# Xiaoming-Zhao/PointNav-VO

Measured on AMD Instinct MI355X. Metric: RGB-D frame-pair VO inferences/s @341x192, higher is better.
Workload: dtype f32

## Files before the change

pointnav-vo_amd/csrc/pnvo_api.hip:

```cpp
#include <hip/hip_runtime.h>

#include <cmath>
#include <cstdio>
#include <cstdlib>
#include <cstring>
#include <functional>
#include <atomic>
#include <condition_variable>
#include <map>
#include <mutex>
#include <string>
#include <thread>
#include <vector>

#include "pnvo_model.h"

using namespace pnvo;

thread_local std::string g_err;

int pnvo_fail(pnvo_handle h, int code, const std::string &msg) {
  if (h) h->err = msg;
  g_err = msg;
  return code;
// ... 432 lines not shown
void pnvo_drop_graphs(pnvo_handle m) {
  for (auto &g : m->graphs) {
    (void)hipGraphExecDestroy(g.exec);
    (void)hipGraphDestroy(g.graph);
  }
  m->graphs.clear();
  m->seen.clear();
}

void pnvo_chain_in_bounds(pnvo_handle h, const std::function<float(const Layer &)> &gn_bound) {
  if (h->bottleneck || h->convs.empty()) return;
  float bin = gn_bound(h->convs[0]);
  size_t li = 1;
  for (int stage = 1; stage <= 4; ++stage)
    for (int bi = 0; bi < h->nblocks[stage - 1]; ++bi) {
      if (li + 1 >= h->convs.size()) return;
      Layer &c1 = h->convs[li++];
      Layer &c2 = h->convs[li++];
      const bool ds = li < h->convs.size() && h->convs[li].name.find("downsample") != std::string::npos;
      c1.in_bound = bin;
      c2.in_bound = gn_bound(c1);
      float skip = bin;
      if (ds) {
        Layer &cd = h->convs[li++];
        cd.in_bound = bin;
        skip = gn_bound(cd);
      }
      bin = gn_bound(c2) + skip;
    }
  if (li < h->convs.size()) h->convs[li].in_bound = bin;
}

bool pnvo_conv_on_x3(pnvo_handle m, const Layer &l, int B) {
  if (!x3_layer(m, l) || l.groups <= 0) return false;
  ConvX3Args xa;
  int mw, nw;
  size_t ldsb;
  return x3_args(m, l, B, xa, &mw, &nw, &ldsb);
}

bool pnvo_conv_takes_ds(pnvo_handle m, const Layer &c1, const Layer &cd, int B) {
  if (!m->opt.ds_fuse || m->tap_dst != nullptr || m->bottleneck) return false;
  if (c1.k != 3 || c1.kw != 3 || c1.stride != 2 || c1.pad != 1 || cd.k != 1 || cd.kw != 1 || cd.stride != 2 || cd.pad != 0) return false;
  if (c1.cinp != cd.cinp || c1.coutp != cd.coutp || c1.cout != cd.cout || c1.hout != cd.hout || c1.wout != cd.wout || c1.hin != cd.hin ||
      c1.win != cd.win || c1.cout != c1.coutp || c1.groups != cd.groups || c1.groups <= 0 || cd.host_w.empty())
    return false;
  if (!x3_layer(m, c1) || !x3_layer(m, cd) || !x3_two_pieces(m, c1) || !x3_two_pieces(m, cd)) return false;
  return pnvo_conv_on_x3(m, c1, B);
}

bool pnvo_conv_takes_tail(pnvo_handle m, const Layer &l, int B) {
  if (m->tap_dst != nullptr || !m->opt.tail) return false;
  return pnvo_conv_on_x3(m, l, B);
}

namespace {
double conv_flops(const Layer &l, int B) { return 2.0 * ((double)((long)B * l.hout * l.wout) * l.cout * l.cin * l.k * l.kw); }
double conv_bytes(const Layer &l, int B) {
  return 4.0 * ((double)B * l.hin * l.win * l.cin + (double)((long)B * l.hout * l.wout) * l.cout + (double)l.cout * l.cin * l.k * l.kw);
}

int x3_operand(pnvo_handle h, Layer &q, int pieces, hipStream_t s) {
  unsigned short *&wpk = pieces == 2 ? q.wpk_x2 : q.wpk_x3;
  unsigned long long &gen = pieces == 2 ? q.x2_gen : q.x3_gen;
  if (wpk && gen == h->weights_gen) return PNVO_OK;
  const size_t nel = (size_t)q.k * q.kw * q.cinp * q.coutp * pieces;
  if (!wpk) HIPCHK(h, hipMalloc((void **)&wpk, nel * 2));
  const float *dev_w = h->train ? pnvo_train_weight_ptr(h, q.name + ".weight") : nullptr;
  if (dev_w != nullptr && pieces == 2) {
    HIPCHK(h, launch_conv_x2_repack(dev_w, q.cout, q.cin, q.cinp, q.coutp, q.k, q.kw, pnvo_train_x2_scale(h, q.name + ".weight"), wpk, s));
  } else if (dev_w != nullptr) {
    HIPCHK(h, launch_conv_x3_repack(dev_w, q.cout, q.cin, q.cinp, q.coutp, q.k, q.kw, 0, wpk, s));
  } else {
    std::vector<unsigned short> pk(nel);
    if (pieces == 2)
      q.x2_oscale = pack_conv_x2_weight(q.host_w.data(), q.cout, q.cin, q.cinp, q.coutp, q.k, q.kw, pk.data());
    else
      pack_conv_x3_weight(q.host_w.data(), q.cout, q.cin, q.cinp, q.coutp, q.k, q.kw, pk.data());
    HIPCHK(h, hipMemcpyAsync(wpk, pk.data(), nel * 2, hipMemcpyHostToDevice, s));
    HIPCHK(h, hipStreamSynchronize(s));
  }
  gen = h->weights_gen;
  return PNVO_OK;
}

int run_conv_x3(pnvo_handle m, const Layer &l, int B, const ConvRequest &r, ConvX3Args &xa, bool rows, int x3_mode, int mw, int nw,
                size_t ldsb) {
  hipStream_t s = r.s;
  const DsRide *ride = r.ride;
  const bool two = xa.np == 2;
  Layer &lm = const_cast<Layer &>(l);
  if (int rc = x3_operand(m, lm, xa.np, s)) return rc;
  if (ride != nullptr) {
    if (rows || !two || l.stride != 2 || l.k != 3) return fail(m, PNVO_ERR_STATE, "downsample ride on a conv that cannot carry it (" + l.name + ")");
    Layer &dm = const_cast<Layer &>(*ride->cd);
    if (int rc = x3_operand(m, dm, 2, s)) return rc;
    xa.ds_wpk = dm.wpk_x2;
    xa.ds_oscale = dm.x2_oscale;
    if (m->train != nullptr) {
      const float *sp = pnvo_train_x2_scale(m, dm.name + ".weight");
      xa.ds_oscale_ptr = sp ? sp + 1 : nullptr;
    }
    xa.ds_y = ride->y;
    xa.ds_stats = m->stats_ds;
  }
  GnGroup gg{0x7fffffff, 0x7fffffff, {nullptr, nullptr}, {nullptr, nullptr}}, ggd = gg;
// ... 448 lines not shown
    a.CPL = m->CPL;
    a.slots = stem_tiles_x(m->Ws) * stem_tiles_y(m->Hs);
    a.dbg = m->opt.stem_dbg;
    a.lds_pad = m->opt.stem_dbg_pad;
    const double M = (double)B * m->Hs * m->Ws;
    {
      Timed t(m, s, "conv:" + stem.name, 2.0 * M * stem.cout * stem.cin * 49,
              4.0 * ((double)B * c.height * c.width * stem.cin + M * stem.cout + (double)stem.cout * stem.cin * 49));
      HIPCHK(m, launch_stem_lds(a, stem.coutp, s));
    }
    m->stem_slots_out = a.slots;
    if (!skip_finalize) {
      Timed t(m, s, "gn_finalize", 0.0, 0.0);
      HIPCHK(m, launch_gn_finalize(m->stats, B, a.slots, stem.coutp, stem.cout, stem.groups, (long)m->Hs * m->Ws, 1,
                                   stem.gamma, stem.beta, 1e-5f, ss[0], ss[1], s, a.slots, mu_out, rstd_out));
    }
  } else {
    if ((rc = pnvo_run_conv(m, stem, B, {.in_scale = m->stem_sc, .in_shift = m->stem_sh, .y = y, .y_cstride = stem.coutp, .ss = ss,
                                         .mu = mu_out, .rstd = rstd_out, .src = src, .grp = grp, .s = s})) != PNVO_OK)
      return rc;
  }
  return rc;
}

int pnvo_ensure_workspace(pnvo_handle m, int B) { return ensure_workspace(m, B); }

namespace {
struct OptChoice {
  const char *word;
  int value;
};
struct OptDef {
  const char *key, *env;
  int PnvoOptions::*field;
  bool numeric;
  OptChoice choices[7];
};
const OptDef kOptions[] = {
    {"stem", "PNVO_STEM", &PnvoOptions::stem, false, {{"auto", 0}, {"mx", 1}, {"dd", 2}, {"dense", 3}, {nullptr, 0}}},
    {"conv", "PNVO_CONV", &PnvoOptions::conv, false, {{"auto", 0}, {"x3", 1}, {"fp32", 2}, {"generic", 3}, {nullptr, 0}}},
    {"pieces", "PNVO_PIECES", &PnvoOptions::pieces, false, {{"2", 2}, {"3", 3}, {nullptr, 0}}},
    {"stem_form", "PNVO_STEM_FORM", &PnvoOptions::stem_form, false, {{"auto", 0}, {"tiles", 2}, {"resident", 3}, {"fast", 4}, {nullptr, 0}}},
    {"train_pieces", "PNVO_TRAIN_PIECES", &PnvoOptions::train_pieces, false, {{"2", 2}, {"3", 3}, {nullptr, 0}}},
    {"x3_persist", "PNVO_X3_PERSIST", &PnvoOptions::x3_persist, false, {{"on", 1}, {"off", 0}, {nullptr, 0}}},
    {"x3_rows", "PNVO_X3_ROWS", &PnvoOptions::x3_rows, false, {{"on", 1}, {"off", 0}, {nullptr, 0}}},
    {"x3_strip", "PNVO_X3_STRIP", &PnvoOptions::x3_strip, false, {{"on", 1}, {"off", 0}, {nullptr, 0}}},
    {"x3_fine", "PNVO_X3_FINE", &PnvoOptions::x3_fine, false, {{"on", 1}, {"off", 0}, {nullptr, 0}}},
    {"x3_w8", "PNVO_X3_W8", &PnvoOptions::x3_w8, false, {{"on", 1}, {"off", 0}, {nullptr, 0}}},
    {"x3_ksplit", "PNVO_X3_KSPLIT", &PnvoOptions::x3_ksplit, false, {{"on", 1}, {"off", 0}, {nullptr, 0}}},
    {"fc_rows", "PNVO_FC_ROWS", &PnvoOptions::fc_rows, true, {{nullptr, 0}}},
    {"head_fuse", "PNVO_HEAD_FUSE", &PnvoOptions::head_fuse, false, {{"on", 1}, {"off", 0}, {nullptr, 0}}},
    {"ds_fuse", "PNVO_DS_FUSE", &PnvoOptions::ds_fuse, false, {{"on", 1}, {"off", 0}, {nullptr, 0}}},
    {"gn_fuse", "PNVO_GN_FUSE", &PnvoOptions::gn_fuse, false, {{"on", 1}, {"off", 0}, {nullptr, 0}}},
    {"x3_s2", nullptr, &PnvoOptions::x3_s2, false, {{"on", 1}, {"off", 0}, {nullptr, 0}}},
    {"tail", "PNVO_TAIL", &PnvoOptions::tail, false, {{"fused", 1}, {"separate", 0}, {nullptr, 0}}},
    {"pool", "PNVO_POOL", &PnvoOptions::pool, false, {{"fused", 1}, {"separate", 0}, {nullptr, 0}}},
    {"graph", "PNVO_GRAPH", &PnvoOptions::graph, true, {{nullptr, 0}}},
    {"stem_dbg", nullptr, &PnvoOptions::stem_dbg, true, {{nullptr, 0}}},
    {"stem_dbg_pad", nullptr, &PnvoOptions::stem_dbg_pad, true, {{nullptr, 0}}},
    {"wgrad_stem", "PNVO_WGRAD_STEM", &PnvoOptions::wgrad_stem, false, {{"mx", 0}, {"fp32", 1}, {nullptr, 0}}},
    {"wgrad3", "PNVO_WGRAD3", &PnvoOptions::wgrad3, false, {{"x3", 1}, {"fp32", 0}, {nullptr, 0}}},
    {"pool_bwd", "PNVO_POOL_BWD", &PnvoOptions::pool_bwd, false, {{"fused", 1}, {"separate", 0}, {nullptr, 0}}},
    {"dgrad", "PNVO_DGRAD", &PnvoOptions::dgrad, false, {{"phase", 1}, {"masked", 0}, {nullptr, 0}}},
    {"bf16_fuse", nullptr, &PnvoOptions::bf16_fuse, false, {{"on", 1}, {"off", 0}, {nullptr, 0}}},
    {"input_fallback", "PNVO_INPUT_FALLBACK", &PnvoOptions::input_fallback, false, {{"on", 1}, {"off", 0}, {nullptr, 0}}},
    {"small_net", "PNVO_SMALL_NET", &PnvoOptions::small_net, false, {{"on", 1}, {"off", 0}, {nullptr, 0}}},
    {"small_max", "PNVO_SMALL_MAX", &PnvoOptions::small_max, true, {{nullptr, 0}}},
    {"small_coop", "PNVO_SMALL_COOP", &PnvoOptions::small_coop, true, {{nullptr, 0}}},
    {"small_prof", "PNVO_SMALL_PROF", &PnvoOptions::small_prof, true, {{nullptr, 0}}},
};

const OptDef *find_option(const char *key) {
  for (const OptDef &d : kOptions)
    if (std::strcmp(d.key, key) == 0) return &d;
  return nullptr;
}

bool parse_option(const OptDef &d, const char *word, int *out) {
  if (d.numeric) {
    char *end = nullptr;
    const long v = std::strtol(word, &end, 10);
    if (end == word || *end != 0) return false;
    *out = (int)v;
    return true;
  }
  for (const OptChoice *c = d.choices; c->word != nullptr; ++c)
    if (std::strcmp(c->word, word) == 0) {
      *out = c->value;
      return true;
    }
  return false;
}

void env_defaults(pnvo_model_s *m) {
  for (const OptDef &d : kOptions) {
    const char *e = d.env ? std::getenv(d.env) : nullptr;
    int v;
    if (e && parse_option(d, e, &v)) m->opt.*(d.field) = v;
  }
  if (std::getenv("PNVO_X3_S2_OFF")) m->opt.x3_s2 = 0;
  if (std::getenv("PNVO_BF16_NOFUSE")) m->opt.bf16_fuse = 0;
  if (const char *e = std::getenv("PNVO_STEM_DBG")) std::sscanf(e, "%d,%d", &m->opt.stem_dbg, &m->opt.stem_dbg_pad);
}
}


// ... 464 lines not shown
  for (auto &g : m->graphs)
    if (g.B == B && std::memcmp(g.key, key, sizeof(key)) == 0) {
      g.stamp = ++m->graph_clock;
      HIPCHK(m, hipGraphLaunch(g.exec, s));
      HIPCHK(m, hipMemcpyAsync(out, m->out_ws, out_bytes, hipMemcpyDeviceToDevice, s));
      return pnvo_mark_stem(m, s, false);
    }
  bool again = false;
  for (auto &g : m->seen) again = again || (g.B == B && std::memcmp(g.key, key, sizeof(key)) == 0);
  if (!again) {
    pnvo_model_s::GraphEntry sn;
    std::memset(&sn, 0, sizeof(sn));
    std::memcpy(sn.key, key, sizeof(key));
    sn.B = B;
    if (m->seen.size() >= 16) m->seen.erase(m->seen.begin());
    m->seen.push_back(sn);
    return forward_body(m, rgb, depth, dd, tdv, actions, B, out, s, nullptr);
  }
  if (!m->cap_stream) HIPCHK(m, hipStreamCreateWithFlags(&m->cap_stream, hipStreamNonBlocking));
  pnvo_model_s::GraphEntry g;
  std::memcpy(g.key, key, sizeof(key));
  g.B = B;
  g.stamp = ++m->graph_clock;
  HIPCHK(m, hipStreamBeginCapture(m->cap_stream, hipStreamCaptureModeRelaxed));
  rc = forward_body(m, rgb, depth, dd, tdv, actions, B, m->out_ws, m->cap_stream, nullptr);
  const hipError_t ce = hipStreamEndCapture(m->cap_stream, &g.graph);
  if (rc != PNVO_OK) {
    if (ce == hipSuccess && g.graph) (void)hipGraphDestroy(g.graph);
    return rc;
  }
  HIPCHK(m, ce);
  HIPCHK(m, hipGraphInstantiate(&g.exec, g.graph, nullptr, nullptr, 0));
  if (m->graphs.size() >= 8) {
    size_t old = 0;
    for (size_t k = 1; k < m->graphs.size(); ++k)
      if (m->graphs[k].stamp < m->graphs[old].stamp) old = k;
    (void)hipGraphExecDestroy(m->graphs[old].exec);
    (void)hipGraphDestroy(m->graphs[old].graph);
    m->graphs.erase(m->graphs.begin() + (long)old);
  }
  m->graphs.push_back(g);
  HIPCHK(m, hipGraphLaunch(g.exec, s));
  HIPCHK(m, hipMemcpyAsync(out, m->out_ws, out_bytes, hipMemcpyDeviceToDevice, s));
  return pnvo_mark_stem(m, s, false);
}
}

namespace {
int run_fc_head(pnvo_handle m, int B, const float *comp_raw, const float *sc, const float *sh, const int64_t *actions, float *out, hipStream_t s);
bool fc_rows_usable(pnvo_handle m, int B);
int run_fc_rows(pnvo_handle m, pnvo_handle const *grp, const int *end, int ng, int B, const float *comp_raw, const float *sc, const float *sh,
                const int64_t *actions, float *out, hipStream_t s);

int forward_body(pnvo_handle m, const float *rgb, const float *depth, const float *dd, const float *tdv,
                 const int64_t *actions, int B, float *out, hipStream_t s, const GroupedFwd *grp) {
  const pnvo_config &c = m->cfg;
  int rc = PNVO_OK;
  if (m->tap_dst != nullptr && m->tap_name == "input") {
    AssembleArgs a;
    a.src[0] = rgb;
    a.src[1] = depth;
    a.src[2] = dd;
    a.src[3] = tdv;
    a.nsrc[0] = c.n_rgb;
    a.nsrc[1] = c.n_depth;
    a.nsrc[2] = c.n_dd;
    a.nsrc[3] = c.n_tdv;
    a.mean = c.normalize ? m->mean.data() : nullptr;
    a.stdev = m->stdev.data();
    a.C = m->C;
    a.CP = m->CP;
    a.npix = (long)B * c.height * c.width;
    free_dev(m->xin);
    HIPCHK(m, hipMalloc((void **)&m->xin, (size_t)a.npix * m->CP * sizeof(float)));
    a.out = m->xin;
    HIPCHK(m, launch_assemble(a, s));
    if ((rc = maybe_tap(m, "input", m->xin, (size_t)B * c.height * c.width * m->CP, s)) != PNVO_OK) return rc;
  }
  size_t li = 0;
  const Layer &stem = m->convs[li++];
  float *cur = m->bufY[0], *nxt = m->bufY[1];
  const bool pool_fused = !m->bottleneck && pnvo_stem_on_mx(m, false) && m->opt.pool && m->convs.size() > 1 &&
                          stem.coutp == stem.cout && pnvo_conv_takes_tail(m, m->convs[1], B);
  const bool small = !pool_fused && stem_writes_slots(m) && pnvo_small_usable(m, B);
  if (small) {
    const float *src[4] = {rgb, depth, dd, tdv};
    if ((rc = pnvo_run_stem(m, B, src, m->stem_raw, m->ssA, nullptr, nullptr, s, nullptr, false, true, grp)) != PNVO_OK) return rc;
    return pnvo_small_forward(m, B, c.act_embed ? actions : nullptr, out, s);
  }
  {
    const float *src[4] = {rgb, depth, dd, tdv};
    if (pool_fused) {
      Timed t(m, s, "pool_init", 0.0, 4.0 * B * m->Hp * m->Wp * stem.coutp);
      HIPCHK(m, hipMemsetD32Async(reinterpret_cast<hipDeviceptr_t>(nxt), STEM_POOL_INIT, (size_t)B * m->Hp * m->Wp * stem.coutp, s));
    }
    if ((rc = pnvo_run_stem(m, B, src, m->stem_raw, m->ssA, nullptr, nullptr, s, pool_fused ? reinterpret_cast<int *>(nxt) : nullptr, false,
                            false, grp)) != PNVO_OK)
      return rc;
  }
  if ((rc = maybe_tap(m, "stem_conv", m->stem_raw, (size_t)B * m->Hs * m->Ws * stem.coutp, s)) != PNVO_OK) return rc;
  if (!pool_fused) {
    Timed t(m, s, "gn_relu_maxpool", 0.0, 4.0 * B * ((double)m->Hs * m->Ws + (double)m->Hp * m->Wp) * stem.coutp);
    HIPCHK(m, launch_gn_relu_maxpool(m->stem_raw, m->ssA[0], m->ssA[1], B, m->Hs, m->Ws, stem.coutp, cur, s));
  }
  if ((rc = maybe_tap(m, "maxpool", cur, (size_t)B * m->Hp * m->Wp * stem.coutp, s)) != PNVO_OK) return rc;

  BlockTail tail{};
  bool have_tail = false, have_keys = pool_fused;
  for (int stage = 1; stage <= 4; ++stage) {
    for (int bi = 0; bi < m->nblocks[stage - 1]; ++bi) {
      if (m->bottleneck) {
        const Layer &b1 = m->convs[li++];
        const Layer &b2 = m->convs[li++];
        const Layer &b3 = m->convs[li++];
        const bool dsb = (li < m->convs.size() && m->convs[li].name.find("downsample") != std::string::npos);
        if ((rc = pnvo_run_conv(m, b1, B, {.x = cur, .y = m->rawA, .y_cstride = b1.coutp, .ss = m->ssA, .grp = grp, .s = s})) != PNVO_OK ||
            (rc = pnvo_run_conv(m, b2, B, {.x = m->rawA, .in_scale = m->ssA[0], .in_shift = m->ssA[1], .y = m->rawC, .y_cstride = b2.coutp,
                                           .ss = m->ssB, .grp = grp, .s = s})) != PNVO_OK ||
            (rc = pnvo_run_conv(m, b3, B, {.x = m->rawC, .in_scale = m->ssB[0], .in_shift = m->ssB[1], .y = m->rawB, .y_cstride = b3.coutp,
                                           .ss = m->ssA, .grp = grp, .s = s})) != PNVO_OK)
          return rc;
        const long Pb = (long)b3.hout * b3.wout;
        if (dsb) {
          const Layer &cd = m->convs[li++];
          if ((rc = pnvo_run_conv(m, cd, B, {.x = cur, .y = m->rawD, .y_cstride = cd.coutp, .ss = m->ssD, .grp = grp, .s = s})) != PNVO_OK)
            return rc;
          Timed t(m, s, "residual", 0.0, 12.0 * B * Pb * b3.coutp);
          HIPCHK(m, launch_residual(m->rawB, m->ssA[0], m->ssA[1], m->rawD, m->ssD[0], m->ssD[1], B, Pb, b3.coutp, nxt, s));
        } else {
          Timed t(m, s, "residual", 0.0, 12.0 * B * Pb * b3.coutp);
          HIPCHK(m, launch_residual(m->rawB, m->ssA[0], m->ssA[1], cur, nullptr, nullptr, B, Pb, b3.coutp, nxt, s));
        }
        std::swap(cur, nxt);
        const std::string tnb = "layer" + std::to_string(stage) + "." + std::to_string(bi);
        if ((rc = maybe_tap(m, tnb.c_str(), cur, (size_t)B * Pb * b3.coutp, s)) != PNVO_OK) return rc;
        continue;
      }
      const Layer &c1 = m->convs[li++];
      const Layer &c2 = m->convs[li++];
      const bool ds = (li < m->convs.size() && m->convs[li].name.find("downsample") != std::string::npos);
      const bool ds_ride = ds && !have_keys && pnvo_conv_takes_ds(m, c1, m->convs[li], B);
      const DsRide ride{ds_ride ? &m->convs[li] : nullptr, m->rawD, m->ssD, nullptr, nullptr};
      if (have_keys) {
        BlockTail ktail{nullptr, nullptr, nullptr, cur};
        if ((rc = pnvo_run_conv(m, c1, B, {.x = nxt, .in_scale = m->ssA[0], .in_shift = m->ssA[1], .y = m->rawA, .y_cstride = c1.coutp,
                                           .ss = m->ssA, .tail = &ktail, .grp = grp, .s = s})) != PNVO_OK)
          return rc;
        have_keys = false;
      } else if (have_tail) {
        if (ds_ride) tail.out = nullptr;
        if ((rc = pnvo_run_conv(m, c1, B, {.x = m->rawB, .in_scale = m->ssB[0], .in_shift = m->ssB[1], .y = m->rawA, .y_cstride = c1.coutp,
                                           .ss = m->ssA, .tail = &tail, .ride = ds_ride ? &ride : nullptr, .grp = grp, .s = s})) != PNVO_OK)
          return rc;
        std::swap(cur, nxt);
        have_tail = false;
      } else if ((rc = pnvo_run_conv(m, c1, B, {.x = cur, .y = m->rawA, .y_cstride = c1.coutp, .ss = m->ssA, .ride = ds_ride ? &ride : nullptr,
                                                .grp = grp, .s = s})) != PNVO_OK) {
        return rc;
      }
      const long P = (long)c2.hout * c2.wout;
      const bool c2_small_generic = !layer_on_lds(m, c2, nullptr) && !pnvo_conv_on_x3(m, c2, B) && (size_t)B * P * c2.cinp * 4 <= ((size_t)48 << 20);
      if (c2_small_generic) {
        float *napp = ds_ride ? nxt : m->rawD;
        {
          Timed t(m, s, "gn_relu_apply", 0.0, 8.0 * B * P * c2.cinp);
          HIPCHK(m, launch_apply_ss_relu(m->rawA, m->ssA[0], m->ssA[1], B, P, c2.cinp, napp, s));
        }
        if ((rc = pnvo_run_conv(m, c2, B, {.x = napp, .y = m->rawB, .y_cstride = c2.coutp, .ss = m->ssB, .grp = grp, .s = s})) != PNVO_OK)
          return rc;
      } else if ((rc = pnvo_run_conv(m, c2, B, {.x = m->rawA, .in_scale = m->ssA[0], .in_shift = m->ssA[1], .y = m->rawB, .y_cstride = c2.coutp,
                                                .ss = m->ssB, .grp = grp, .s = s})) != PNVO_OK) {
        return rc;
      }
      if (ds) {
        const Layer &cd = m->convs[li++];
        if (!ds_ride &&
            (rc = pnvo_run_conv(m, cd, B, {.x = cur, .y = m->rawD, .y_cstride = cd.coutp, .ss = m->ssD, .grp = grp, .s = s})) != PNVO_OK)
          return rc;
      }
      if (li < m->convs.size() && pnvo_conv_takes_tail(m, m->convs[li], B)) {
        tail.res = ds ? m->rawD : cur;
        tail.res_scale = ds ? m->ssD[0] : nullptr;
        tail.res_shift = ds ? m->ssD[1] : nullptr;
        tail.out = nxt;
        have_tail = true;
        continue;
      }
      {
        Timed t(m, s, "residual", 0.0, 12.0 * B * P * c2.coutp);
        HIPCHK(m, launch_residual(m->rawB, m->ssB[0], m->ssB[1], ds ? m->rawD : cur, ds ? m->ssD[0] : nullptr, ds ? m->ssD[1] : nullptr, B,
                                  P, c2.coutp, nxt, s));
      }
      std::swap(cur, nxt);
      const std::string tn = "layer" + std::to_string(stage) + "." + std::to_string(bi);
      if ((rc = maybe_tap(m, tn.c_str(), cur, (size_t)B * P * c2.coutp, s)) != PNVO_OK) return rc;
    }
  }

  const Layer &comp = m->convs[li++];
  if (have_tail) {
    tail.out = nullptr;
    if ((rc = pnvo_run_conv(m, comp, B, {.x = m->rawB, .in_scale = m->ssB[0], .in_shift = m->ssB[1], .y = m->comp_raw, .y_cstride = comp.coutp,
                                         .ss = m->ssC, .tail = &tail, .grp = grp, .s = s})) != PNVO_OK)
      return rc;
    have_tail = false;
  } else if ((rc = pnvo_run_conv(m, comp, B, {.x = cur, .y = m->comp_raw, .y_cstride = comp.coutp, .ss = m->ssC, .grp = grp, .s = s})) != PNVO_OK) {
    return rc;
  }
  if (m->tap_dst != nullptr && m->tap_name == "compression") {
    HIPCHK(m, launch_apply_ss_relu(m->comp_raw, m->ssC[0], m->ssC[1], B, (long)m->fh * m->fw, m->comp_cp, m->tapbuf, s));
    if ((rc = maybe_tap(m, "compression", m->tapbuf, (size_t)B * m->fh * m->fw * m->comp_cp, s)) != PNVO_OK) return rc;
  }
// ... 644 lines not shown
```

pointnav-vo_amd/csrc/pnvo_internal.h:

```cpp
#pragma once
#include <mutex>
#include <hip/hip_runtime.h>
#include <stdint.h>

namespace pnvo {

constexpr int PNVO_ABSMAX_UINTS = 64 * 16;

struct SrcPiece {
  const float *base;
  int nch;
  int choff;
};

struct ConvArgs {
  const float *x;
  const float *wpk;
  float *y;
  const float *in_scale;
  const float *in_shift;
  float *stats;
  const float *bias;
  const int64_t *bias_row;
  int B, H, W, CIN;
// ... 113 lines not shown
  int np;
  float oscale;
  const float *oscale_ptr;
  int persist_wgs;
  int w8_ok, w8;
  int ksw_ok, ksw;
  int fine;
  int strip;
  const float *gn_gamma, *gn_beta;
  float *gn_scale, *gn_shift;
  float *gn_mu, *gn_rstd;
  int gn_cpg;
  float gn_eps;
  long gn_P;
  const unsigned short *ds_wpk;
  float *ds_y, *ds_stats;
  float ds_oscale;
  const float *ds_oscale_ptr;
  const float *ds_gamma, *ds_beta;
  float *ds_scale, *ds_shift;
  float *ds_mu, *ds_rstd;
  int grp_end0, grp_end1;
  const unsigned short *wpk_g[2], *ds_wpk_g[2];
  float oscale_g[2], ds_oscale_g[2];
  const float *gn_gamma_g[2], *gn_beta_g[2], *ds_gamma_g[2], *ds_beta_g[2];
};
#if defined(__HIPCC__)
__device__ __forceinline__ void gn_finalize_lane(float s1, float s2, int cpg, long P, float eps, float gamma, float beta, float *scale, float *shift,
                                                 float *mu_out = nullptr, float *rstd_out = nullptr) {
#pragma clang fp contract(off)
  double d1 = (double)s1, d2 = (double)s2;
  for (int o = cpg >> 1; o >= 1; o >>= 1) {
    d1 += __shfl_xor(d1, o);
    d2 += __shfl_xor(d2, o);
  }
  const double cnt = (double)P * cpg;
  const double mu = d1 / cnt;
  double var = d2 / cnt - mu * mu;
  if (var < 0.0) var = 0.0;
  const double rstd = 1.0 / sqrt(var + (double)eps);
  if (mu_out != nullptr) {
    *mu_out = (float)mu;
    *rstd_out = (float)rstd;
  }
  const double sc = rstd * (double)gamma;
  *scale = (float)sc;
  *shift = (float)((double)beta - mu * sc);
}
#endif
bool conv_x3_plan(ConvX3Args &a, int ks, int stride, int *mw, int *nw, size_t *lds_bytes);
bool conv_rows32_plan(ConvX3Args &a, int ks, int stride, int mode, int num_cus);
hipError_t launch_conv_rows32(const ConvX3Args &a, int mode, int num_cus, hipStream_t s);
hipError_t launch_conv_x3(const ConvX3Args &a, int ks, int stride, int mode, int mw, int nw, size_t lds_bytes, hipStream_t s);
hipError_t launch_conv_x3_repack(const float *w_oihw, int cout, int cin, int cinp, int coutp, int kh, int kw, int transposed,
                                 unsigned short *out, hipStream_t s);
void pack_conv_x3_weight(const float *oihw, int cout, int cin, int cinp, int coutp, int kh, int kw, unsigned short *out);
hipError_t launch_conv_x2_scales(const float *params, const long *seg_dev, int nseg, float *out, hipStream_t s);
hipError_t launch_conv_x2_repack(const float *w_oihw, int cout, int cin, int cinp, int coutp, int kh, int kw, const float *scale_dev,
                                 unsigned short *out, hipStream_t s, int transposed = 0);
float pack_conv_x2_weight(const float *oihw, int cout, int cin, int cinp, int coutp, int kh, int kw, unsigned short *out);

struct ConvBArgs {
  const unsigned short *x[2];
  const unsigned short *wpk[2];
  void *y[2];
  const float *in_scale[2], *in_shift[2];
  const unsigned short *x2[2];
  const float *in_scale2[2], *in_shift2[2];
  unsigned short *xout[2];
  float *stats[2];
  int B, H, W, CIN, Ho, Wo, COUTP;
  int TR, TC, tiles_r, tiles_c, PR, PC, CK, MT, wn, slots;
  int persist_wgs;
  const unsigned short *ds_wpk[2];
  void *ds_y[2];
  float *ds_stats[2];
  const float *ds_gamma[2], *ds_beta[2];
  float *ds_scale[2], *ds_shift[2];
  const float *gn_gamma[2], *gn_beta[2];
  float *gn_scale[2], *gn_shift[2];
  int gn_cpg;
  float gn_eps;
  long gn_P;
};
bool conv_bf16_plan(ConvBArgs &a, int ks, int stride, int *mw, int *nw, size_t *lds_bytes);
hipError_t launch_conv_bf16(const ConvBArgs &a, int ks, int stride, int mode, bool f32out, int mw, int nw, size_t lds_bytes,
                            int nmodels, hipStream_t s);
void pack_conv_bf16_weight(const float *oihw, int cout, int cin, int cinp, int coutp, int kh, int kw, unsigned short *out);
hipError_t launch_gn_relu_maxpool_bf16(const unsigned short *const *x, const float *const *scale, const float *const *shift,
                                       int B, int H, int W, int C, unsigned short *const *out, int nmodels, hipStream_t s);
hipError_t launch_residual_bf16(const unsigned short *const *a, const float *const *sa, const float *const *ta,
                                const unsigned short *const *b, const float *const *sb, const float *const *tb, int B, long P,
                                int C, unsigned short *const *y, int nmodels, hipStream_t s);

int conv_slots(int P, int MT);
void choose_tile(long M, int COUTP, int *MT, int *NT);
hipError_t launch_conv(const ConvArgs &a, hipStream_t s);
hipError_t launch_ksplit_reduce(const ConvArgs &a, hipStream_t s);
constexpr int FC_ROWS_MAXV = 12;
struct FcRowsArgs {
  const float *x, *sc, *sh;
  float *hid, *out;
  const int64_t *actions;
  int B, Kp, cp, hidden, out_dim, ngroups;
  int end[3];
  const float *w[3], *bias[3], *head_w[3], *head_b[3];
// ... 179 lines not shown
```

pointnav-vo_amd/csrc/pnvo_model.h:

```cpp
#pragma once
#include <hip/hip_runtime.h>

#include <map>
#include <functional>
#include <string>
#include <vector>

#include "../../include/pnvo.h"
#include "pnvo_internal.h"

static inline int rup(int x, int m) { return (x + m - 1) / m * m; }
static inline int halve(int x) { return (x - 1) / 2 + 1; }

struct Layer {
  std::string name, gn;
  int cin = 0, cinp = 0, cout = 0, coutp = 0, k = 1, kw = 1, stride = 1, pad = 0;
  int hin = 0, win = 0, hout = 0, wout = 0, groups = 1;
  float *wpk = nullptr, *gamma = nullptr, *beta = nullptr;
  std::vector<float> host_w;
  unsigned short *wpk_x3 = nullptr;
  unsigned long long x3_gen = 0;
  unsigned short *wpk_x2 = nullptr;
  unsigned long long x2_gen = 0;
  float x2_oscale = 1.f;
  float in_bound = 3.0e38f;
};

struct PnvoOptions {
  int stem = 0;
  int conv = 0;
  int stem_form = 0;
  int pieces = 2;
  int train_pieces = 2;
  int x3_rows = 1;
  int x3_persist = 1;
  int x3_strip = 1;
  int x3_fine = 1;
  int x3_w8 = 1;
  int x3_ksplit = 1;
  int fc_rows = 48;
  int head_fuse = 1;
  int ds_fuse = 1;
  int gn_fuse = 1;
  int x3_s2 = 1;
  int tail = 1;
  int pool = 1;
  int graph = 0;
  int stem_dbg = 0, stem_dbg_pad = 0;
  int wgrad_stem = 0;
  int wgrad3 = 1;
  int pool_bwd = 1;
  int dgrad = 1;
  int bf16_fuse = 1;
  int input_fallback = 1;
  int small_net = 1;
  int small_max = 3;
  int small_prof = 0;
  int small_coop = 1;
};

struct TimingRec {
  hipEvent_t a, b;
  int entry;
};

struct pnvo_model_s {
  pnvo_config cfg;
  int device = 0;
  std::string err;
  std::string note;
  bool loaded = false;

  int C = 0, CP = 0;
  int Hs = 0, Ws = 0, Hp = 0, Wp = 0, fh = 0, fw = 0, comp_c = 0, comp_cp = 0;
  std::vector<Layer> convs;
  Layer fc, head;
  float *fc_bias = nullptr, *head_bias = nullptr;
  float *fc_rows_w = nullptr;
  float *head_w_plain = nullptr;
  std::vector<float> mean, stdev;
  std::vector<int> stem_ref_of_new;
  std::vector<int> stem_tensor_of_new, stem_ch_of_new;
  float *stem_sc = nullptr, *stem_sh = nullptr, *zero_page = nullptr;
  float *kpart = nullptr;
  size_t kpart_floats = 0;
  float *stem_wpk16 = nullptr;
  int CPL = 0;
  bool dd_ok = false;
  int dd_bins = 0;
  std::vector<int> dd_dense_tensor, dd_dense_ch;
  float *dd_wpk = nullptr, *dd_table = nullptr, *dd_sc = nullptr, *dd_sh = nullptr;
  int *dd_flag = nullptr;
  int *dd_flag_dev = nullptr;
  unsigned long long *dd_prof = nullptr;

  bool mx_ok = false;
// ... 62 lines not shown
  int graph_mode = -1;
  unsigned long long graph_clock = 0;

  int timing = 0;
  std::vector<pnvo_kernel_time> tentries;
  std::map<std::string, int> tindex;
  std::vector<TimingRec> trecs;
  std::vector<hipEvent_t> evpool;
};


struct BlockTail {
  const float *res, *res_scale, *res_shift;
  float *out;
};

struct DsRide {
  const Layer *cd;
  float *y;
  float *const *ss;
  float *mu, *rstd;
};

struct GroupedFwd {
  int n;
  pnvo_model_s *h[3];
  int end[3];
};

struct ConvRequest {
  const float *x = nullptr;
  const float *in_scale = nullptr, *in_shift = nullptr;
  float *y = nullptr;
  int y_cstride = 0;
  float *const *ss = nullptr;
  float *mu = nullptr, *rstd = nullptr;
  const float *bias = nullptr;
  const int64_t *bias_row = nullptr;
  int relu_out = 0;
  const float *const *src = nullptr;
  const BlockTail *tail = nullptr;
  const DsRide *ride = nullptr;
  const GroupedFwd *grp = nullptr;
  const float *head_w = nullptr;
  float *head_out = nullptr;
  bool *head_rode = nullptr;
  hipStream_t s = nullptr;
};

int pnvo_run_conv(pnvo_handle m, const Layer &l, int B, const ConvRequest &r);
bool pnvo_conv_takes_ds(pnvo_handle m, const Layer &c1, const Layer &cd, int B);
bool pnvo_conv_on_x3(pnvo_handle m, const Layer &l, int B);
bool pnvo_conv_takes_tail(pnvo_handle m, const Layer &l, int B);
void pnvo_pack_conv_weight_cinp(const float *oihw, int cout, int cin, int cinp, int kh, int kw, std::vector<float> &out);
int pnvo_run_stem(pnvo_handle m, int B, const float *const *src, float *y, float *const *ss, float *mu_out, float *rstd_out,
                  hipStream_t s, int *pool_keys, bool train_fwd, bool skip_finalize, const GroupedFwd *grp);
bool pnvo_stem_on_mx(pnvo_handle m, bool train_fwd);
void pnvo_stem_raw_args(pnvo_handle m, pnvo::StemMXArgs &a);
int pnvo_mark_stem(pnvo_handle m, hipStream_t s, bool train_fwd);
int pnvo_input_fallback(pnvo_handle m, hipStream_t s, bool *rerun);
void pnvo_train_free(pnvo_handle m);
const float *pnvo_train_weight_ptr(pnvo_handle m, const std::string &name);
void pnvo_chain_in_bounds(pnvo_handle h, const std::function<float(const Layer &)> &gn_bound);
const float *pnvo_train_x2_scale(pnvo_handle m, const std::string &name);
void pnvo_bf16_free(pnvo_handle m);
bool pnvo_small_usable(pnvo_handle m, int B);
int pnvo_small_forward(pnvo_handle m, int B, const int64_t *actions, float *out, hipStream_t s);
void pnvo_small_free(pnvo_handle m);
int pnvo_forward_bf16(pnvo_handle *hs, int nm, const float *rgb, const float *depth, const float *dd, const float *tdv,
                      const int64_t *actions, int B, float *const *outs, hipStream_t s);
int pnvo_fail(pnvo_handle h, int code, const std::string &msg);
void pnvo_free_dev(float *&p);
int pnvo_ensure_workspace(pnvo_handle m, int B);
void pnvo_drop_graphs(pnvo_handle m);

#define HIPCHK(h, expr)                                                                                   \
  do {                                                                                                    \
    hipError_t e__ = (expr);                                                                              \
    if (e__ != hipSuccess)                                                                                \
      return pnvo_fail(h, PNVO_ERR_HIP, std::string(#expr) + ": " + hipGetErrorString(e__));             \
  } while (0)

struct PnvoTimed {
  pnvo_model_s *m;
  hipStream_t s;
  int rec = -1;
  PnvoTimed(pnvo_model_s *m_, hipStream_t s_, const std::string &name, double flops, double bytes);
  ~PnvoTimed();
};
```

Before: 112,600.

## Fuse ResNet stage-4 tail convs and compression into one persistent kernel

Adds a single per-sample kernel that runs the remaining three stage-4 3x3 convs, their GroupNorm, residual adds, and the compression conv with its GN statistics. Activations stay resident in LDS as split f16 pairs, so there is no global round-trip between layers and far fewer launches. The kernel is gated on a narrow shape check and is on by default. The trade-off is one workgroup per sample, which may underuse the GPU at small batch, plus a large LDS footprint.

```diff
diff --git a/pointnav-vo_amd/csrc/pnvo_api.hip b/pointnav-vo_amd/csrc/pnvo_api.hip
--- a/pointnav-vo_amd/csrc/pnvo_api.hip
+++ b/pointnav-vo_amd/csrc/pnvo_api.hip
@@ -508,6 +508,36 @@
 bool pnvo_conv_takes_tail(pnvo_handle m, const Layer &l, int B) {
   if (m->tap_dst != nullptr || !m->opt.tail) return false;
   return pnvo_conv_on_x3(m, l, B);
+}
+
+bool pnvo_stage4_takes(pnvo_handle m, int B) {
+  if (!m->opt.stage4 || m->bottleneck || m->train != nullptr || m->tap_dst != nullptr || m->opt.conv != 0 || m->opt.pieces != 2) return false;
+  if (m->nblocks.size() != 4 || m->nblocks[3] != 2 || m->convs.size() < 7) return false;
+  const size_t N = m->convs.size();
+  const Layer &hd = m->convs[N - 6], &cd = m->convs[N - 4], &cp = m->convs[N - 1];
+  const Layer *cv[3] = {&m->convs[N - 5], &m->convs[N - 3], &m->convs[N - 2]};
+  if (hd.name.find("layer4.0.convs.0") == std::string::npos || cd.name.find("layer4.0.downsample") == std::string::npos ||
+      cp.name.find("compression") == std::string::npos || hd.cout != 256 || hd.coutp != 256 || cd.coutp != 256)
+    return false;
+  const int P = hd.hout * hd.wout;
+  if (P <= 64 || P > 96 || cd.hout != hd.hout || cd.wout != hd.wout) return false;
+  for (const Layer *c : cv) {
+    const int cpg = c->groups > 0 ? c->cout / c->groups : 0;
+    if (c->k != 3 || c->kw != 3 || c->stride != 1 || c->pad != 1 || c->cin != 256 || c->cinp != 256 || c->cout != 256 || c->coutp != 256 ||
+        c->hin != hd.hout || c->win != hd.wout || c->hout != hd.hout || c->wout != hd.wout || cpg < 1 || cpg > 32 || 32 % cpg != 0 ||
+        c->cout % cpg != 0 || !x3_layer(m, *c) || !x3_two_pieces(m, *c))
+      return false;
+  }
+  if (cp.k != 3 || cp.kw != 3 || cp.stride != 1 || cp.pad != 1 || cp.cinp != 256 || cp.coutp != 32 || cp.cout > 32 || cp.groups != 1 ||
+      cp.hin != hd.hout || cp.win != hd.wout || cp.hout != hd.hout || cp.wout != hd.wout || !x3_layer(m, cp) || !x3_two_pieces(m, cp))
+    return false;
+  ConvX3Args xa;
+  x3_fill(m, *cv[0], B, xa);
+  xa.w8_ok = 1;
+  xa.fine = 0;
+  int mw = 0, nw = 0;
+  size_t ldsb = 0;
+  return conv_x3_plan(xa, 3, 1, &mw, &nw, &ldsb) && xa.w8 == 1 && xa.tiles_r * xa.tiles_c == 1 && xa.CK == 128;
 }
 
 namespace {
@@ -1062,6 +1092,7 @@
     {"head_fuse", "PNVO_HEAD_FUSE", &PnvoOptions::head_fuse, false, {{"on", 1}, {"off", 0}, {nullptr, 0}}},
     {"ds_fuse", "PNVO_DS_FUSE", &PnvoOptions::ds_fuse, false, {{"on", 1}, {"off", 0}, {nullptr, 0}}},
     {"gn_fuse", "PNVO_GN_FUSE", &PnvoOptions::gn_fuse, false, {{"on", 1}, {"off", 0}, {nullptr, 0}}},
+    {"stage4", "PNVO_STAGE4", &PnvoOptions::stage4, false, {{"on", 1}, {"off", 0}, {nullptr, 0}}},
     {"x3_s2", nullptr, &PnvoOptions::x3_s2, false, {{"on", 1}, {"off", 0}, {nullptr, 0}}},
     {"tail", "PNVO_TAIL", &PnvoOptions::tail, false, {{"fused", 1}, {"separate", 0}, {nullptr, 0}}},
     {"pool", "PNVO_POOL", &PnvoOptions::pool, false, {{"fused", 1}, {"separate", 0}, {nullptr, 0}}},
@@ -1632,10 +1663,52 @@
 int run_fc_rows(pnvo_handle m, pnvo_handle const *grp, const int *end, int ng, int B, const float *comp_raw, const float *sc, const float *sh,
                 const int64_t *actions, float *out, hipStream_t s);
 
+static int run_stage4(pnvo_handle m, int B, hipStream_t s) {
+  const size_t N = m->convs.size();
+  Layer *cv[3] = {&m->convs[N - 5], &m->convs[N - 3], &m->convs[N - 2]};
+  Layer &cp = m->convs[N - 1];
+  Stage4Args a;
+  std::memset(&a, 0, sizeof(a));
+  a.xa = m->rawA;
+  a.xa_scale = m->ssA[0];
+  a.xa_shift = m->ssA[1];
+  a.xd = m->rawD;
+  a.xd_scale = m->ssD[0];
+  a.xd_shift = m->ssD[1];
+  double flops = 0.0;
+  for (int k = 0; k < 3; ++k) {
+    if (int rc = x3_operand(m, *cv[k], 2, s)) return rc;
+    a.wpk[k] = cv[k]->wpk_x2;
+    a.oscale[k] = cv[k]->x2_oscale;
+    a.gamma[k] = cv[k]->gamma;
+    a.beta[k] = cv[k]->beta;
+    a.cpg[k] = cv[k]->cout / cv[k]->groups;
+    flops += conv_flops(*cv[k], B);
+  }
+  if (int rc = x3_operand(m, cp, 2, s)) return rc;
+  a.cwpk = cp.wpk_x2;
+  a.coscale = cp.x2_oscale;
+  a.cgamma = cp.gamma;
+  a.cbeta = cp.beta;
+  a.cC = cp.cout;
+  a.cy = m->comp_raw;
+  a.cscale = m->ssC[0];
+  a.cshift = m->ssC[1];
+  a.B = B;
+  a.Ho = cp.hout;
+  a.Wo = cp.wout;
+  flops += conv_flops(cp, B);
+  const double P = (double)cp.hout * cp.wout;
+  Timed t(m, s, "stage4", flops, 4.0 * B * P * (2.0 * 256 + 32) + 2.0 * 4.0 * 9 * 256 * (3 * 256 + 32));
+  HIPCHK(m, launch_stage4(a, s));
+  return PNVO_OK;
+}
+
 int forward_body(pnvo_handle m, const float *rgb, const float *depth, const float *dd, const float *tdv,
                  const int64_t *actions, int B, float *out, hipStream_t s, const GroupedFwd *grp) {
   const pnvo_config &c = m->cfg;
   int rc = PNVO_OK;
+  const bool s4 = grp == nullptr && pnvo_stage4_takes(m, B);
   if (m->tap_dst != nullptr && m->tap_name == "input") {
     AssembleArgs a;
     a.src[0] = rgb;
@@ -1738,6 +1811,13 @@
                                                 .grp = grp, .s = s})) != PNVO_OK) {
         return rc;
       }
+      if (s4 && stage == 4 && bi == 0) {
+        if (ds && !ds_ride && (rc = pnvo_run_conv(m, m->convs[li], B, {.x = cur, .y = m->rawD, .y_cstride = m->convs[li].coutp, .ss = m->ssD,
+                                                                       .s = s})) != PNVO_OK)
+          return rc;
+        if ((rc = run_stage4(m, B, s)) != PNVO_OK) return rc;
+        return run_fc_head(m, B, m->comp_raw, m->ssC[0], m->ssC[1], actions, out, s);
+      }
       const long P = (long)c2.hout * c2.wout;
       const bool c2_small_generic = !layer_on_lds(m, c2, nullptr) && !pnvo_conv_on_x3(m, c2, B) && (size_t)B * P * c2.cinp * 4 <= ((size_t)48 << 20);
       if (c2_small_generic) {
diff --git a/pointnav-vo_amd/csrc/pnvo_internal.h b/pointnav-vo_amd/csrc/pnvo_internal.h
--- a/pointnav-vo_amd/csrc/pnvo_internal.h
+++ b/pointnav-vo_amd/csrc/pnvo_internal.h
@@ -189,6 +189,24 @@
 bool conv_rows32_plan(ConvX3Args &a, int ks, int stride, int mode, int num_cus);
 hipError_t launch_conv_rows32(const ConvX3Args &a, int mode, int num_cus, hipStream_t s);
 hipError_t launch_conv_x3(const ConvX3Args &a, int ks, int stride, int mode, int mw, int nw, size_t lds_bytes, hipStream_t s);
+struct Stage4Args {
+  const float *xa, *xa_scale, *xa_shift;
+  const float *xd, *xd_scale, *xd_shift;
+  const unsigned short *wpk[3];
+  float oscale[3];
+  const float *gamma[3], *beta[3];
+  int cpg[3];
+  const unsigned short *cwpk;
+  float coscale;
+  const float *cgamma, *cbeta;
+  int cC;
+  float *cy;
+  float *cscale, *cshift;
+  int B, Ho, Wo;
+  unsigned long long *prof;
+};
+size_t stage4_lds_bytes(int Ho, int Wo);
+hipError_t launch_stage4(const Stage4Args &a, hipStream_t s);
 hipError_t launch_conv_x3_repack(const float *w_oihw, int cout, int cin, int cinp, int coutp, int kh, int kw, int transposed,
                                  unsigned short *out, hipStream_t s);
 void pack_conv_x3_weight(const float *oihw, int cout, int cin, int cinp, int coutp, int kh, int kw, unsigned short *out);
diff --git a/pointnav-vo_amd/csrc/pnvo_model.h b/pointnav-vo_amd/csrc/pnvo_model.h
--- a/pointnav-vo_amd/csrc/pnvo_model.h
+++ b/pointnav-vo_amd/csrc/pnvo_model.h
@@ -42,6 +42,7 @@
   int head_fuse = 1;
   int ds_fuse = 1;
   int gn_fuse = 1;
+  int stage4 = 1;
   int x3_s2 = 1;
   int tail = 1;
   int pool = 1;
@@ -210,6 +211,7 @@
 bool pnvo_conv_takes_ds(pnvo_handle m, const Layer &c1, const Layer &cd, int B);
 bool pnvo_conv_on_x3(pnvo_handle m, const Layer &l, int B);
 bool pnvo_conv_takes_tail(pnvo_handle m, const Layer &l, int B);
+bool pnvo_stage4_takes(pnvo_handle m, int B);
 void pnvo_pack_conv_weight_cinp(const float *oihw, int cout, int cin, int cinp, int kh, int kw, std::vector<float> &out);
 int pnvo_run_stem(pnvo_handle m, int B, const float *const *src, float *y, float *const *ss, float *mu_out, float *rstd_out,
                   hipStream_t s, int *pool_keys, bool train_fwd, bool skip_finalize, const GroupedFwd *grp);
diff --git a/pointnav-vo_amd/csrc/stage4.hip b/pointnav-vo_amd/csrc/stage4.hip
--- /dev/null
+++ b/pointnav-vo_amd/csrc/stage4.hip
@@ -0,0 +1,360 @@
+#include <algorithm>
+#include <cmath>
+#include <cstdio>
+#include <cstdlib>
+#include <cstring>
+
+#include "pnvo_internal.h"
+
+namespace pnvo {
+
+namespace {
+typedef float f32x16 __attribute__((ext_vector_type(16)));
+typedef float f32x4 __attribute__((ext_vector_type(4)));
+typedef float f32x2 __attribute__((ext_vector_type(2)));
+typedef _Float16 f16x8 __attribute__((ext_vector_type(8)));
+typedef _Float16 f16x2 __attribute__((ext_vector_type(2)));
+typedef unsigned u32x4 __attribute__((ext_vector_type(4)));
+
+constexpr int S4_C = 256;
+constexpr int S4_PITCH = S4_C * 2 + 16;
+constexpr int S4_MT = 3;
+constexpr int S4_CK = 128;
+constexpr int S4_KCC = S4_CK / 16;
+constexpr int S4_NSTEPS = 9 * S4_KCC;
+
+__device__ __forceinline__ void s4_gn_one_group(float s1, float s2, int lane, int C, long P, float eps, const float *gamma, const float *beta,
+                                                float *scale, float *shift) {
+#pragma clang fp contract(off)
+  double d1 = 0.0, d2 = 0.0;
+  if (lane < C) {
+    d1 += (double)s1;
+    d2 += (double)s2;
+  }
+#pragma unroll
+  for (int o = 32; o >= 1; o >>= 1) {
+    d1 += __shfl_xor(d1, o);
+    d2 += __shfl_xor(d2, o);
+  }
+  const double cnt = (double)P * C;
+  const double mu = d1 / cnt;
+  double var = d2 / cnt - mu * mu;
+  if (var < 0.0) var = 0.0;
+  const double rstd = 1.0 / sqrt(var + (double)eps);
+  if (lane < C) {
+    const double sc = rstd * (double)gamma[lane];
+    scale[lane] = (float)sc;
+    shift[lane] = (float)((double)beta[lane] - mu * sc);
+  }
+}
+
+template <int NTT>
+__device__ __forceinline__ void s4_kloop(f32x16 (&acc)[S4_MT], const unsigned char *lds, int plane, const unsigned (&aoff)[S4_MT],
+                                         const unsigned short *wpk, int nt, int lane, int PC, int t0, int t1) {
+  constexpr unsigned kstep = (unsigned)NTT * 2048u;
+  const unsigned voff = (unsigned)nt * 2048u + (unsigned)lane * 16u;
+#pragma unroll 1
+  for (int h = 0; h < S4_C / S4_CK; ++h) {
+    const int tap = t0 / S4_KCC;
+    int kc_n = t0 - tap * S4_KCC, kw_n = tap % 3;
+    unsigned toff_n = (unsigned)(((tap / 3) * PC + kw_n) * S4_PITCH + h * S4_CK * 2 + kc_n * 32);
+    const char *wb_n = reinterpret_cast<const char *>(wpk) + (long)(tap * (S4_C / 16) + h * S4_KCC + kc_n) * kstep;
+    auto advance = [&]() {
+      ++kc_n;
+      toff_n += 32;
+      wb_n += kstep;
+      if (kc_n == S4_KCC) {
+        kc_n = 0;
+        toff_n += (unsigned)(S4_PITCH - S4_KCC * 32);
+        wb_n += (long)(S4_C / 16 - S4_KCC) * kstep;
+        if (++kw_n == 3) {
+          kw_n = 0;
+          toff_n += (unsigned)((PC - 3) * S4_PITCH);
+        }
+      }
+    };
+    auto loadA = [&](int i, u32x4 (*a)[S4_MT]) {
+#pragma unroll
+      for (int pc = 0; pc < 2; ++pc) a[pc][i] = *reinterpret_cast<const u32x4 *>(lds + pc * plane + aoff[i] + toff_n);
+    };
+    auto loadB = [&](u32x4 *b) {
+#pragma unroll
+      for (int pc = 0; pc < 2; ++pc) b[pc] = *reinterpret_cast<const u32x4 *>(wb_n + voff + pc * 1024);
+    };
+    auto step = [&](u32x4 (*a)[S4_MT], const u32x4 *b) {
+#pragma unroll
+      for (int i = 0; i < S4_MT; ++i) {
+        constexpr int TA[3] = {1, 0, 0}, TB[3] = {0, 1, 0};
+#pragma unroll
+        for (int t = 0; t < 3; ++t)
+          acc[i] = __builtin_amdgcn_mfma_f32_32x32x16_f16(__builtin_bit_cast(f16x8, a[TA[t]][i]), __builtin_bit_cast(f16x8, b[TB[t]]), acc[i], 0, 0, 0);
+        __builtin_amdgcn_sched_barrier(0);
+        loadA(i, a);
+        __builtin_amdgcn_sched_barrier(0);
+      }
+    };
+    u32x4 a[2][S4_MT], b0[2], b1[2];
+    loadB(b0);
+#pragma unroll
+    for (int i = 0; i < S4_MT; ++i) loadA(i, a);
+    advance();
+#pragma unroll 1
+    for (int t = t0; t < t1; t += 2) {
+      const bool more = t + 2 < t1;
+      loadB(b1);
+      __builtin_amdgcn_sched_barrier(0);
+      step(a, b0);
+      if (more) advance();
+      loadB(b0);
+      __builtin_amdgcn_sched_barrier(0);
+      step(a, b1);
+      if (more) advance();
+    }
+  }
+}
+
+__device__ __forceinline__ int s4_row(int i, int r, int lane) { return i * 32 + 8 * (r >> 2) + 4 * (lane >> 5) + (r & 3); }
+}
+
+__global__ __launch_bounds__(512) __attribute__((amdgpu_waves_per_eu(2, 2))) void stage4_kernel(const Stage4Args p) {
+  extern __shared__ __attribute__((aligned(16))) unsigned char lds[];
+  const int lane = threadIdx.x & 63;
+  const int wave = __builtin_amdgcn_readfirstlane(threadIdx.x >> 6);
+  const int chunk = (p.B + 7) >> 3;
+  const int n = (int)(blockIdx.x & 7) * chunk + (int)(blockIdx.x >> 3);
+  if (n >= p.B) return;
+  if (wave >= 4) __builtin_amdgcn_s_setprio(1);
+  const int Wo = p.Wo, P = p.Ho * p.Wo, PC = Wo + 2;
+  const int plane = (p.Ho + 2) * PC * S4_PITCH;
+  unsigned *qtab = reinterpret_cast<unsigned *>(lds + 2 * plane);
+  const unsigned ctr = (unsigned)((PC + 1) * S4_PITCH);
+  unsigned long long *prof = p.prof != nullptr && lane == 0 && blockIdx.x == 13 ? p.prof + wave * 12 : nullptr;
+  unsigned long long t_prev = __builtin_readcyclecounter();
+  const unsigned long long t_0 = t_prev;
+  auto mark = [&](int k) {
+    const unsigned long long t = __builtin_readcyclecounter();
+    if (prof != nullptr) prof[k] = t - t_prev;
+    t_prev = t;
+  };
+
+  {
+    const u32x4 z = {0u, 0u, 0u, 0u};
+    for (int e = (int)threadIdx.x; e < 2 * plane / 16; e += 512) *reinterpret_cast<u32x4 *>(lds + 16 * e) = z;
+    for (int e = (int)threadIdx.x; e < S4_MT * 32; e += 512) {
+      const int q = min(e, P - 1);
+      const int tr = q / Wo, tc = q - tr * Wo;
+      qtab[e] = (unsigned)((tr * PC + tc) * S4_PITCH);
+    }
+  }
+  const int ch = wave * 32 + (lane & 31);
+  const long sbase = (long)n * P * S4_C;
+  float xs[S4_MT][16];
+  {
+    const float rs = p.xd_scale[(long)n * S4_C + ch], rt = p.xd_shift[(long)n * S4_C + ch];
+    float raw[S4_MT][16];
+#pragma unroll
+    for (int i = 0; i < S4_MT; ++i)
+#pragma unroll
+      for (int r = 0; r < 16; ++r) {
+        const int q = s4_row(i, r, lane);
+        raw[i][r] = q < P ? p.xd[sbase + (long)q * S4_C + ch] : 0.f;
+      }
+#pragma unroll
+    for (int i = 0; i < S4_MT; ++i)
+#pragma unroll
+      for (int r = 0; r < 16; ++r) xs[i][r] = __builtin_fmaf(raw[i][r], rs, rt);
+  }
+  __syncthreads();
+  {
+    const int cg = threadIdx.x & 31, pl = threadIdx.x >> 5;
+    const float *ps = p.xa_scale + (long)n * S4_C + 8 * cg, *pt = p.xa_shift + (long)n * S4_C + 8 * cg;
+    const f32x4 sc0 = *reinterpret_cast<const f32x4 *>(ps), sc1 = *reinterpret_cast<const f32x4 *>(ps + 4);
+    const f32x4 sh0 = *reinterpret_cast<const f32x4 *>(pt), sh1 = *reinterpret_cast<const f32x4 *>(pt + 4);
+    constexpr int R = (S4_MT * 32) / 16;
+    f32x4 v[R][2];
+#pragma unroll
+    for (int k = 0; k < R; ++k) {
+      const int q = pl + 16 * k;
+      v[k][0] = v[k][1] = f32x4{0.f, 0.f, 0.f, 0.f};
+      if (q < P) {
+        const float *src = p.xa + sbase + (long)q * S4_C + 8 * cg;
+        v[k][0] = *reinterpret_cast<const f32x4 *>(src);
+        v[k][1] = *reinterpret_cast<const f32x4 *>(src + 4);
+      }
+    }
+#pragma unroll
+    for (int k = 0; k < R; ++k) {
+      const int q = pl + 16 * k;
+      if (q >= P) continue;
+      u32x4 o0, o1;
+#pragma unroll
+      for (int e = 0; e < 4; ++e) {
+        float f[2];
+#pragma unroll
+        for (int u = 0; u < 2; ++u) {
+          const int c = 2 * e + u;
+          const f32x4 &sc = c < 4 ? sc0 : sc1, &sh = c < 4 ? sh0 : sh1;
+          f[u] = fmaxf(__builtin_fmaf(v[k][c >> 2][c & 3], sc[c & 3], sh[c & 3]), 0.f);
+        }
+        const f16x2 hh = __builtin_convertvector(f32x2{f[0], f[1]}, f16x2);
+        o0[e] = __builtin_bit_cast(unsigned, hh);
+        o1[e] = __builtin_bit_cast(unsigned, __builtin_convertvector(f32x2{f[0] - (float)hh[0], f[1] - (float)hh[1]}, f16x2));
+      }
+      const unsigned off = qtab[q] + ctr + 16u * (unsigned)cg;
+      *reinterpret_cast<u32x4 *>(lds + off) = o0;
+      *reinterpret_cast<u32x4 *>(lds + plane + off) = o1;
+    }
+  }
+  __syncthreads();
+  mark(0);
+
+  unsigned aoff[S4_MT];
+#pragma unroll
+  for (int i = 0; i < S4_MT; ++i) aoff[i] = qtab[i * 32 + (lane & 31)] + (unsigned)((lane >> 5) * 16);
+  f32x16 acc[S4_MT];
+
+#pragma unroll 1
+  for (int k = 0; k < 3; ++k) {
+#pragma unroll
+    for (int i = 0; i < S4_MT; ++i)
+#pragma unroll
+      for (int r = 0; r < 16; ++r) acc[i][r] = 0.f;
+    s4_kloop<S4_C / 32>(acc, lds, plane, aoff, p.wpk[k], wave, lane, PC, 0, S4_NSTEPS);
+    mark(1 + 2 * k);
+    const float os = p.oscale[k];
+    float t1 = 0.f, t2 = 0.f;
+#pragma unroll
+    for (int i = 0; i < S4_MT; ++i) {
+      float s1 = 0.f, s2 = 0.f;
+#pragma unroll
+      for (int r = 0; r < 16; ++r) {
+        acc[i][r] *= os;
+        const float v = s4_row(i, r, lane) < P ? acc[i][r] : 0.f;
+        s1 += v;
+        s2 = __builtin_fmaf(v, v, s2);
+      }
+      t1 += s1 + __shfl_xor(s1, 32);
+      t2 += s2 + __shfl_xor(s2, 32);
+    }
+    float gsc, gsh;
+    gn_finalize_lane(t1, t2, p.cpg[k], P, 1e-5f, p.gamma[k][ch], p.beta[k][ch], &gsc, &gsh);
+    __syncthreads();
+#pragma unroll
+    for (int i = 0; i < S4_MT; ++i)
+#pragma unroll
+      for (int r = 0; r < 16; ++r) {
+        const int q = s4_row(i, r, lane);
+        const u32x4 qe = *reinterpret_cast<const u32x4 *>(qtab + (q & ~3));
+        float y = __builtin_fmaf(acc[i][r], gsc, gsh);
+        if (k != 1) {
+          y = fmaxf(y + xs[i][r], 0.f);
+          if (k == 0) xs[i][r] = y;
+        } else {
+          y = fmaxf(y, 0.f);
+        }
+        if (q < P) {
+          const _Float16 h0 = (_Float16)y, h1 = (_Float16)(y - (float)h0);
+          const unsigned off = qe[r & 3] + ctr + 2u * (unsigned)ch;
+          *reinterpret_cast<_Float16 *>(lds + off) = h0;
+          *reinterpret_cast<_Float16 *>(lds + plane + off) = h1;
+        }
+      }
+    __syncthreads();
+    mark(2 + 2 * k);
+  }
+
+  if (wave < 4) {
+#pragma unroll
+    for (int i = 0; i < S4_MT; ++i)
+#pragma unroll
+      for (int r = 0; r < 16; ++r) acc[i][r] = 0.f;
+    s4_kloop<1>(acc, lds, plane, aoff, p.cwpk, 0, lane, PC, (wave * S4_NSTEPS) >> 2, ((wave + 1) * S4_NSTEPS) >> 2);
+  }
+  mark(7);
+  __syncthreads();
+  float *part = reinterpret_cast<float *>(lds);
+  if (wave < 4) {
+#pragma unroll
+    for (int i = 0; i < S4_MT; ++i)
+#pragma unroll
+      for (int r = 0; r < 16; ++r) part[((wave * S4_MT + i) * 16 + r) * 64 + lane] = acc[i][r];
+  }
+  __syncthreads();
+  float t1 = 0.f, t2 = 0.f;
+  if (wave < S4_MT) {
+    const float os = p.coscale;
+    float s1 = 0.f, s2 = 0.f;
+    float *y = p.cy + (long)n * P * 32 + (lane & 31);
+#pragma unroll
+    for (int r = 0; r < 16; ++r) {
+      float v = part[((0 * S4_MT + wave) * 16 + r) * 64 + lane];
+#pragma unroll
+      for (int w = 1; w < 4; ++w) v += part[((w * S4_MT + wave) * 16 + r) * 64 + lane];
+      v *= os;
+      const int q = s4_row(wave, r, lane);
+      if (q < P) y[(long)q * 32] = v;
+      v = q < P ? v : 0.f;
+      s1 += v;
+      s2 = __builtin_fmaf(v, v, s2);
+    }
+    t1 += s1 + __shfl_xor(s1, 32);
+    t2 += s2 + __shfl_xor(s2, 32);
+  }
+  float *red = reinterpret_cast<float *>(lds + 4 * S4_MT * 16 * 64 * 4);
+  if (wave < 4 && lane < 32) *reinterpret_cast<f32x2 *>(red + (wave * 32 + lane) * 2) = f32x2{t1, t2};
+  __syncthreads();
+  if (wave == 0) {
+    float s1 = t1, s2 = t2;
+    for (int w = 1; w < 4; ++w) {
+      const f32x2 o = *reinterpret_cast<const f32x2 *>(red + (w * 32 + (lane & 31)) * 2);
+      s1 += o[0];
+      s2 += o[1];
+    }
+    s4_gn_one_group(s1, s2, lane, p.cC, P, 1e-5f, p.cgamma, p.cbeta, p.cscale + (long)n * 32, p.cshift + (long)n * 32);
+  }
+  mark(8);
+  if (prof != nullptr) prof[9] = __builtin_readcyclecounter() - t_0;
+}
+
+hipError_t launch_stage4(const Stage4Args &a0, hipStream_t s) {
+  Stage4Args a = a0;
+  if (a.Ho * a.Wo <= 64 || a.Ho * a.Wo > S4_MT * 32 || a.cC < 1 || a.cC > 32) return hipErrorInvalidValue;
+  const size_t ldsb = stage4_lds_bytes(a.Ho, a.Wo);
+  if (ldsb > (size_t)160 * 1024) return hipErrorInvalidValue;
+  static bool attr = false;
+  if (!attr) {
+    hipError_t e = hipFuncSetAttribute(reinterpret_cast<const void *>(stage4_kernel), hipFuncAttributeMaxDynamicSharedMemorySize, 160 * 1024);
+    if (e != hipSuccess) return e;
+    attr = true;
+  }
+  static unsigned long long *prof = nullptr;
+  static const bool want = std::getenv("PNVO_S4_PROF") != nullptr;
+  if (want && !prof) {
+    (void)hipMalloc((void **)&prof, 8 * 12 * 8);
+    (void)hipMemset(prof, 0, 8 * 12 * 8);
+  }
+  a.prof = prof;
+  hipLaunchKernelGGL(stage4_kernel, dim3((unsigned)(((a.B + 7) / 8) * 8)), dim3(512), ldsb, s, a);
+  hipError_t e = hipGetLastError();
+  if (prof && e == hipSuccess) {
+    static int calls = 0;
+    if (++calls <= 40) {
+      unsigned long long h[8 * 12];
+      (void)hipStreamSynchronize(s);
+      (void)hipMemcpy(h, prof, sizeof(h), hipMemcpyDeviceToHost);
+      for (int w = 0; w < 8; w += 4)
+        std::fprintf(stderr, "[pnvo] stage4 B %d %dx%d wave%d: stage %llu | conv0 k %llu x %llu | conv1 k %llu x %llu | conv2 k %llu x %llu | "
+                             "comp k %llu epi %llu | total %llu\n", a.B, a.Ho, a.Wo, w, h[w * 12 + 0], h[w * 12 + 1], h[w * 12 + 2], h[w * 12 + 3],
+                     h[w * 12 + 4], h[w * 12 + 5], h[w * 12 + 6], h[w * 12 + 7], h[w * 12 + 8], h[w * 12 + 9]);
+    }
+  }
+  return e;
+}
+
+size_t stage4_lds_bytes(int Ho, int Wo) {
+  const size_t planes = (size_t)2 * (Ho + 2) * (Wo + 2) * S4_PITCH;
+  const size_t reduce = (size_t)4 * S4_MT * 16 * 64 * 4 + 4 * 32 * 2 * 4;
+  return std::max(planes, reduce) + (size_t)S4_MT * 32 * 4;
+}
+
+}
```

After: 114,000, median of 6. No clear change (+1.2%).
